# aluo-x/3D_SLN

Measured on AMD Instinct MI355X. Metric: scene-graph VAE steps/sec + 256² diff-render fps, 1/2/4/8 MI355X, higher is better.
Workload: dtype f32; 1 GPU; BASELINE configs[1]: batch=64 scene graphs x (32 objects, 64 triples) per GPU, Sg2ScVAE train step at train.py defaults (embedding_dim=64, 5+5 GraphTripleConv, BatchNorm); O=2048, T=4096, hipgraph=True, distinct_batches_cycled=4, eps=N(0,1) drawn on the device inside the step, parallelism=dp1

## Files before the change

### 3d_sln_amd/_lib.py

```python
from __future__ import annotations

import ctypes as C
import os

HERE = os.path.dirname(os.path.abspath(__file__))
LIB_PATH = os.path.join(HERE, "libsln_hip.so")

SLN_E = {-1: "SLN_E_BADARG", -2: "SLN_E_UNSUPPORTED", -3: "SLN_E_STATE", -4: "SLN_E_NOGPU", -5: "SLN_E_NOMEM", -6: "SLN_E_CAPTURE"}

c_f32p = C.c_void_p
c_i64p = C.c_void_p


class SlnError(RuntimeError):
    pass


class SlnVaeConfig(C.Structure):
    _fields_ = [(n, C.c_int) for n in (
        "embedding_dim", "gconv_num_layers", "recurrent", "batch_norm", "decoder_cat", "use_ae",
        "box_dim", "n_angle", "num_objs", "num_preds", "num_attrs", "no_attr")]


class SlnVaeUnit(C.Structure):
# ... 49 lines not shown
    _fields_ = [("P", SlnPlacement)] + \
               [(n, C.c_void_p) for n in ("boxes", "angles", "size_target", "faces_out", "sizes", "size_loss", "grad_faces", "grad_size_loss",
                                          "grad_boxes", "grad_angles", "boxes_pred", "angles_pred", "noise", "noise_step")] + \
               [("noise_stride", C.c_int64)] + [(n, C.c_void_p) for n in ("box_last", "angle_last", "grad_boxes_pred", "grad_angles_pred")] + \
               [("n_angle", C.c_int), ("ld_gb", C.c_int), ("beta", C.c_float), ("pad_", C.c_int)]


class SlnVaeGroupIO(C.Structure):
    _fields_ = [("rows_total", C.c_int), ("row0_host", C.POINTER(C.c_int))] + \
               [(n, C.c_void_p) for n in ("z", "boxes_pred", "angles_pred", "d_boxes_pred", "d_angles_pred", "dz", "sgd_step")]


class SlnDbgBn(C.Structure):
    _fields_ = [(n, C.c_void_p) for n in ("sums", "gsums", "gamma", "beta", "rmean", "rvar")] + \
               [("cstride", C.c_int), ("mode", C.c_int), ("n_rows", C.c_float), ("eps", C.c_float)]


class SlnDbgSeg(C.Structure):
    _fields_ = [("x1", C.c_void_p), ("x2", C.c_void_p)] + \
               [(n, C.c_int) for n in ("ld1", "ld2", "c1", "c2", "len", "which", "coef", "pad_")] + [("bn", SlnDbgBn)]


class SlnDbgOperand(C.Structure):
    _fields_ = [("seg", SlnDbgSeg * 3), ("idx_a", C.c_void_p), ("idx_b", C.c_void_p), ("nseg", C.c_int), ("pad_", C.c_int)]


class SlnDbgGemmNT(C.Structure):
    _fields_ = [("A", SlnDbgOperand)] + [(n, C.c_void_p) for n in ("W", "bias", "Y", "addend", "xprev", "osums", "ogsums")] + \
               [("obn", SlnDbgBn)] + \
               [(n, C.c_int) for n in ("M", "N", "K", "ldw", "ldy", "ycol0", "ldadd", "addcol0", "ocstride", "ldx", "xcol0", "epi", "tile",
                                       "pad_")]


class SlnDbgGemmTN(C.Structure):
    _fields_ = [("G", SlnDbgOperand), ("X", SlnDbgOperand), ("dW", C.c_void_p), ("db", C.c_void_p), ("sgd_step", C.c_void_p)] + \
               [(n, C.c_int) for n in ("lddw", "R", "Nout", "Kin", "rows_per_block", "pad_")]


class SlnDbgNTRoute(C.Structure):
    _fields_ = [(n, C.c_int) for n in ("body", "multi", "amode", "threads")]


SIGNATURES = {
    "sln_version": (C.c_int, []),
    "sln_build_arch": (C.c_char_p, []),
    "sln_device_ok": (C.c_int, []),
    "sln_vae_num_units": (C.c_int, [C.POINTER(SlnVaeConfig)]),
    "sln_vae_create": (C.c_int, [C.POINTER(SlnVaeConfig), C.POINTER(C.c_void_p)]),
    "sln_vae_destroy": (None, [C.c_void_p]),
    "sln_vae_workspace_bytes": (C.c_int64, [C.c_void_p, C.c_int, C.c_int]),
    "sln_vae_bind": (C.c_int, [C.c_void_p, C.POINTER(SlnVaeTensors), C.c_void_p, C.c_int64, C.c_int, C.c_int]),
    "sln_vae_set_batch": (C.c_int, [C.c_void_p, C.POINTER(SlnVaeBatch), C.c_void_p]),
    "sln_vae_check_batch": (C.c_int, [C.c_void_p, C.c_void_p]),
    "sln_vae_encoder": (C.c_int, [C.c_void_p, c_f32p, c_f32p, C.c_int, C.c_void_p]),
    "sln_vae_decoder": (C.c_int, [C.c_void_p, c_f32p, c_f32p, c_f32p, C.c_int, C.c_void_p]),
    "sln_vae_forward": (C.c_int, [C.c_void_p, c_f32p, c_f32p, c_f32p, c_f32p, c_f32p, c_f32p, C.c_int, C.c_void_p]),
    "sln_vae_loss": (C.c_int, [C.c_void_p, c_f32p, c_f32p, c_f32p, c_f32p, C.c_float, c_f32p, C.c_int, C.c_void_p]),
    "sln_vae_decoder_backward": (C.c_int, [C.c_void_p, c_f32p, c_f32p, c_f32p, C.c_void_p]),
    "sln_vae_encoder_backward": (C.c_int, [C.c_void_p, c_f32p, c_f32p, C.c_void_p]),
    "sln_vae_backward": (C.c_int, [C.c_void_p, C.c_void_p]),
    "sln_vae_params_changed": (C.c_int, [C.c_void_p]),
    "sln_vae_zero_grad": (C.c_int, [C.c_void_p, C.c_void_p]),
    "sln_vae_adam_step": (C.c_int, [C.c_void_p, C.c_float, C.c_void_p]),
    "sln_vae_adam_reset": (C.c_int, [C.c_void_p, C.c_int64, C.c_void_p]),
    "sln_vae_adam_get_step": (C.c_int, [C.c_void_p, C.POINTER(C.c_int64), C.c_void_p]),
    "sln_vae_set_grad_guard": (C.c_int, [C.c_void_p, c_f32p]),
    "sln_vae_seed": (C.c_int, [C.c_void_p, C.c_uint64, C.c_uint64, C.c_void_p]),
    "sln_vae_last_eps": (C.c_int, [C.c_void_p, c_f32p, C.c_void_p]),
    "sln_vae_randn": (C.c_int, [C.c_void_p, c_f32p, C.c_int64, C.c_void_p]),
    "sln_layout_heatmap": (C.c_int, [c_f32p, C.c_int64, C.c_int, C.c_int, C.c_int, C.c_int, c_f32p, C.c_void_p]),
    "sln_vae_set_training": (C.c_int, [C.c_void_p, C.c_int]),
    "sln_vae_train_step": (C.c_int, [C.c_void_p, c_f32p, C.c_float, C.c_float, c_f32p, C.c_int, C.c_int, C.c_void_p]),
    "sln_vae_group_create": (C.c_int, [C.POINTER(C.c_void_p), C.c_int, C.POINTER(SlnVaeGroupIO), C.POINTER(C.c_void_p)]),
    "sln_vae_group_decoder": (C.c_int, [C.c_void_p, C.c_void_p]),
    "sln_vae_group_decoder_backward": (C.c_int, [C.c_void_p, C.c_void_p]),
    "sln_vae_group_launches": (C.c_int, [C.c_void_p, C.POINTER(C.c_int), C.POINTER(C.c_int), C.POINTER(C.c_int)]),
    "sln_vae_group_transposes": (C.c_int64, [C.c_void_p]),
    "sln_vae_group_fused_params": (C.c_int, [C.c_void_p, C.POINTER(C.c_void_p), C.POINTER(C.c_int64), C.c_int]),
    "sln_vae_group_destroy": (None, [C.c_void_p]),
    "sln_debug_side_stream": (C.c_int, [C.c_void_p, C.POINTER(C.c_int), C.POINTER(C.c_int)]),
    "sln_side_stream_prepare": (C.c_int, [C.c_void_p]),
    "sln_side_stream_forget": (C.c_int, [C.c_void_p]),
    "sln_prof_enable": (C.c_int, [C.c_int]),
    "sln_set_deterministic": (C.c_int, [C.c_int]),
    "sln_get_deterministic": (C.c_int, []),
    "sln_debug_tn_plan": (C.c_int, [C.c_void_p, C.c_void_p, C.c_void_p, C.c_int, C.c_void_p, C.c_void_p, C.c_int]),
    "sln_prof_read": (C.c_int, [C.c_void_p, C.c_void_p, C.c_void_p, C.c_int]),
    "sln_vae_tap": (C.c_int64, [C.c_void_p, C.c_int, C.c_int, c_f32p, C.c_void_p]),
    "sln_gconv_workspace_bytes": (C.c_int64, [C.c_int, C.c_int, C.c_int, C.c_int, C.c_int, C.c_int]),
    "sln_gconv_forward": (C.c_int, [C.c_int, C.c_int, C.c_int, C.c_int, C.c_int, C.c_int, C.POINTER(SlnVaeUnit), c_f32p, c_f32p,
                                    C.c_void_p, C.c_int, C.c_int, C.c_int, C.c_void_p, C.c_int64, c_f32p, c_f32p, C.c_void_p]),
    "sln_gconv_net_create": (C.c_int, [C.c_int, C.c_int, C.c_int, C.c_int, C.c_int, C.c_int, C.POINTER(C.c_void_p)]),
    "sln_gconv_net_set_edges": (C.c_int, [C.c_void_p, C.c_void_p, C.c_int, C.c_int, C.c_void_p]),
    "sln_gconv_net_forward": (C.c_int, [C.c_void_p, c_f32p, c_f32p, c_f32p, c_f32p, C.c_int, C.c_void_p]),
    "sln_gconv_net_backward": (C.c_int, [C.c_void_p, c_f32p, c_f32p, c_f32p, c_f32p, C.c_void_p]),
    "sln_linear_forward": (C.c_int, [c_f32p, C.c_int, C.c_int, c_f32p, c_f32p, c_f32p, C.c_int, C.c_void_p,
                                     C.c_int, C.c_void_p]),
    "sln_linear_wgrad": (C.c_int, [c_f32p, c_f32p, C.c_int, C.c_int, C.c_int, c_f32p, c_f32p, C.c_void_p]),
    "sln_debug_gemm_nt": (C.c_int, [C.POINTER(SlnDbgGemmNT), C.c_int, C.POINTER(C.c_int), C.c_void_p]),
    "sln_debug_gemm_tn": (C.c_int, [C.POINTER(SlnDbgGemmTN), C.c_int, C.c_int, C.c_void_p]),
    "sln_debug_gemm_nt_route": (C.c_int, [C.POINTER(SlnDbgGemmNT), C.POINTER(SlnDbgNTRoute)]),
    "sln_debug_gemm_sizes": (C.c_int, [C.POINTER(C.c_int), C.c_int]),
    "sln_project_faces": (C.c_int, [c_f32p, C.c_void_p, c_f32p, c_f32p, c_f32p, C.c_int, C.c_int, C.c_int, C.c_float, C.c_float, c_f32p, C.c_void_p]),
    "sln_project_faces_backward": (C.c_int, [c_f32p, C.c_void_p, c_f32p, c_f32p, c_f32p, C.c_int, C.c_int, C.c_int, C.c_float, C.c_float, c_f32p,
                                             c_f32p, C.c_void_p]),
    "sln_raster_workspace_bytes": (C.c_int64, [C.c_int, C.c_int]),
# ... 143 lines not shown
```

### 3d_sln_amd/csrc/vae_engine.hip

```cpp
#include <cstddef>
#include <new>
#include <type_traits>
#include <utility>
#include <vector>
#include <cstring>
#include <cstdlib>

#include "../../include/sln_hip.h"
#include "sln_gemm.h"
#include "vae_kernels.h"
#include "vae_multi.h"
#include "sln_prof.h"

namespace {

enum { SK_DEC_ASSEMBLE = 0, SK_EMBED_GATHER, SK_NT, SK_SCATTER_FWD, SK_TN, SK_TN_FLUSH, SK_MASK_GSTATS, SK_ADD2, SK_EMBED_BWD,
       SK_SCATTER_BWD, SK_GATHER_BWD, SK_DEC_ASSEMBLE_BWD, SK_COPY2D };
struct RecStep {
  int kind = -1, epi = 0, idx64 = 0;
  GemmNTArgs nt; GemmTNArgs tn;
  MScatterFwd sf; MScatterBwd sb; MGatherBwd gb; MMaskGstats mg; MDecAssemble da; DecAssembleBwd dab; MEmbedGather eg; MEmbedBwd eb; MAdd2 a2;
};
struct Recorder { std::vector<RecStep> steps; };

// ... 32 lines not shown
struct Bump {
  char* base; size_t off = 0; bool dry;
  explicit Bump(void* b) : base(static_cast<char*>(b)), dry(b == nullptr) {}
  template <typename T> T* take(size_t n) {
    off = (off + 255) & ~size_t(255);
    T* p = dry ? nullptr : reinterpret_cast<T*>(base + off);
    off += n * sizeof(T);
    return p;
  }
};

}

struct SlnVae {
  SlnVaeConfig cfg;
  int E, H, L, nmod, n_obj_e, n_attr_e, n_box_e, n_angle_e, Dec, Ddc;
  std::vector<Unit> units;
  SlnVaeTensors t;
  bool bound = false;
  int maxO = 0, maxT = 0, O = 0, T = 0;
  SlnVaeBatch batch;
  bool batch_set = false;

  std::vector<Layer> layers;
  std::vector<BnInst> bns;
  int bn_head[6] = {-1, -1, -1, -1, -1, -1};
  int n_bn_enc = 0;

  GraphCsr g;
  int* attrs32 = nullptr; int* err_flag = nullptr;
  double* stats_base = nullptr; size_t stats_doubles = 0, enc_stats_doubles = 0;
  double* gstats_base = nullptr;
  char* zero_begin = nullptr; size_t zero_bytes = 0; bool bulk_zeroed = false;
  bool step_training = true;
  int64_t* st_objs = nullptr; int64_t* st_angles = nullptr; int64_t* st_attrs = nullptr; float* st_boxes = nullptr;
  BnTableEntry* bn_table_dev = nullptr;
  TransposeEntry* tr_table_dev = nullptr; int n_tr = 0, tr_max_tiles = 0;
  AdamScalars* scalars = nullptr; double* loss_acc = nullptr; float* losses = nullptr;
  float *X0e = nullptr, *P0e = nullptr, *X0d = nullptr, *P0d = nullptr;
  float *hbA1 = nullptr, *hbA2 = nullptr, *haA1 = nullptr, *haA2 = nullptr;
  float *mu = nullptr, *logvar = nullptr, *z = nullptr, *eps_buf = nullptr;
  float *bnA1 = nullptr, *anA1 = nullptr, *boxes_pred = nullptr, *logits = nullptr, *angles_pred = nullptr;
  float *dbp = nullptr, *dlogits = nullptr, *g_bn = nullptr, *g_an = nullptr, *d_bx = nullptr, *d_ax = nullptr;
  float *dM = nullptr, *dG[2] = {nullptr, nullptr};
  float *dX0 = nullptr, *dz = nullptr, *dmu = nullptr, *dlv = nullptr;
  float *g_h2 = nullptr, *g_h1 = nullptr, *d_xb = nullptr, *d_xa = nullptr, *tmp_d = nullptr;
  float *g_h2b = nullptr, *g_h1b = nullptr, *tmp_db = nullptr;
  int dbp_ld = 8;

  bool enc_training = false, dec_training = false, have_enc = false, have_dec = false, have_loss_grads = false;
  const float* z_src = nullptr;
  bool z_from_latent = false;
  bool wt_fresh = false;
  float host_kl = 0.f, host_lr = 0.f; int64_t host_step = 0; bool host_scalars_valid = false;
  float* grad_guard = nullptr;
  bool draw_eps = false;
  unsigned long long host_seed[2] = {0, 0};

  struct TnGroup {
    GemmTNArgs probs[SLN_TN_MULTI_MAX]; TnMultiMeta meta; int n = 0, blocks = 0; bool x2 = false, xg = false; double flops = 0.0;
    bool dirty = true; GemmTNArgs* dev_probs = nullptr; TnMultiMeta* dev_meta = nullptr;
  };
  int tn_slots = 32;
  std::vector<GemmTNArgs> tn_kind_scratch;
  bool capturing = false, tn_upload_pending = false;
  int det_seen = 0;
  bool tn_per_layer = false;
  int tn_slot_next[3] = {0, 0, 0};
  std::vector<GemmTNArgs> deferred;
  TnGroup* tn_groups_store = nullptr;
  TnGroup& tn_group(int set, int slot, int k) { return tn_groups_store[((size_t)set * tn_slots + slot) * 2 + k]; }
  int upload_group(TnGroup& g) {
    hipError_t e = hipMemcpy(g.dev_probs, g.probs, sizeof(GemmTNArgs) * (size_t)g.n, hipMemcpyHostToDevice);
    if (e == hipSuccess) e = hipMemcpy(g.dev_meta, &g.meta, sizeof(TnMultiMeta), hipMemcpyHostToDevice);
    g.dirty = e != hipSuccess;
    return (int)e;
  }
  bool bn_table_live = false;
  struct TnStage { char* host = nullptr; hipEvent_t done = nullptr; };
  enum { TN_STAGE_SLOTS = 16 };
  TnStage tn_stage[TN_STAGE_SLOTS];
  int tn_stage_next = 0;
  int stage_upload(void* dev0, const void* src0, size_t n0, void* dev1, const void* src1, size_t n1, hipStream_t st) {
    hipStreamCaptureStatus cs = hipStreamCaptureStatusNone;
    if (hipStreamIsCapturing(st, &cs) != hipSuccess || cs != hipStreamCaptureStatusNone) return SLN_E_CAPTURE;
    const size_t cap0 = sizeof(GemmTNArgs) * (size_t)SLN_TN_MULTI_MAX, cap = cap0 + sizeof(TnMultiMeta);
    if (n0 > cap0 || n1 > cap - cap0) return SLN_E_BADARG;
    TnStage& sl = tn_stage[tn_stage_next];
    tn_stage_next = (tn_stage_next + 1) % TN_STAGE_SLOTS;
    hipError_t e = hipSuccess;
    if (!sl.host) {
      void* hp = nullptr;
      if (hipHostMalloc(&hp, cap, hipHostMallocDefault) != hipSuccess) return SLN_E_NOMEM;
      sl.host = static_cast<char*>(hp);
      if (hipEventCreateWithFlags(&sl.done, hipEventDisableTiming) != hipSuccess) { (void)hipHostFree(hp); sl.host = nullptr; return SLN_E_NOMEM; }
    } else {
      e = hipEventSynchronize(sl.done);
    }
    if (e == hipSuccess && n0) { std::memcpy(sl.host, src0, n0); e = hipMemcpyAsync(dev0, sl.host, n0, hipMemcpyHostToDevice, st); }
    if (e == hipSuccess && n1) { std::memcpy(sl.host + cap0, src1, n1); e = hipMemcpyAsync(dev1, sl.host + cap0, n1, hipMemcpyHostToDevice, st); }
    if (e == hipSuccess) e = hipEventRecord(sl.done, st);
    return (int)e;
  }
  int upload_group_async(TnGroup& g, hipStream_t st) {
    const int r = stage_upload(g.dev_probs, g.probs, sizeof(GemmTNArgs) * (size_t)g.n, g.dev_meta, &g.meta,
                               offsetof(TnMultiMeta, item) + sizeof(TnMultiItem) * (size_t)g.meta.nblocks, st);
// ... 834 lines not shown
  }
  h->n_tr = (int)tr.size(); h->tr_max_tiles = maxt;
  HIP_RET(hipMemcpy(h->tr_table_dev, tr.data(), sizeof(TransposeEntry) * tr.size(), hipMemcpyHostToDevice));
  AdamScalars sc; std::memset(&sc, 0, sizeof(sc));
  sc.step = 0; sc.lr = 1e-4f; sc.beta1 = 0.9f; sc.beta2 = 0.999f; sc.eps = 1e-8f; sc.kl_weight = 0.1f; sc.bc1 = 1.f; sc.bc2 = 1.f;
  sc.rng_seed = h->host_seed[0]; sc.rng_offset = h->host_seed[1];
  HIP_RET(hipMemcpy(h->scalars, &sc, sizeof(sc), hipMemcpyHostToDevice));
  RET_IF(sln_gemm_init());
  h->host_scalars_valid = false;
  h->bound = true; h->batch_set = false; h->wt_fresh = false; h->have_enc = h->have_dec = false; h->bn_table_live = false;
  h->drop_graphs();
  return 0;
}

static int upload_bn_table(SlnVae* h) {
  std::vector<BnTableEntry> tab(h->bns.size());
  for (size_t i = 0; i < h->bns.size(); ++i) {
    BnInst& b = h->bns[i];
    const Unit& u = h->units[b.unit];
    BnTableEntry e; std::memset(&e, 0, sizeof(e));
    e.sums = b.sums; e.gsums = b.gsums; e.cstride = b.C; e.C = b.C; e.rows = b.rows_code;
    e.rmean = u.p.bn_running_mean; e.rvar = u.p.bn_running_var; e.nbt = u.p.bn_num_batches_tracked;
    e.dgamma = u.p.d_bn_weight; e.dbeta = u.p.d_bn_bias;
    tab[i] = e;
  }
  if (!tab.empty()) HIP_RET(hipMemcpy(h->bn_table_dev, tab.data(), sizeof(BnTableEntry) * tab.size(), hipMemcpyHostToDevice));
  return 0;
}

int sln_vae_set_batch(SlnVae* h, const SlnVaeBatch* b, void* stream) {
  if (!h || !b || !h->bound) return SLN_E_BADARG;
  if (b->O <= 0 || b->T < 0 || b->O > h->maxO || b->T > h->maxT) return SLN_E_BADARG;
  if (!b->objs || !b->boxes || !b->angles || !b->attributes || (b->T > 0 && !b->triples)) return SLN_E_BADARG;
  hipStream_t st = (hipStream_t)stream;
  const bool shape_changed = (b->O != h->O) || (b->T != h->T) || !h->batch_set;
  h->batch = *b; h->O = b->O; h->T = b->T;
  h->g.T = b->T; h->g.O = b->O;
  if (shape_changed) {
    for (auto& ly : h->layers)
      for (int k = 0; k < 4; ++k)
        if (ly.bn[k] >= 0) h->bns[ly.bn[k]].rows = k < 2 ? b->T : b->O;
    for (int s = 0; s < 6; ++s)
      if (h->bn_head[s] >= 0) h->bns[h->bn_head[s]].rows = b->O;
    if (!h->bn_table_live) {
      HIP_RET(hipStreamSynchronize(st));
      RET_IF(upload_bn_table(h));
      h->bn_table_live = true;
    }
    bool has_graph = false;
    for (int i = 0; i < 4; ++i) has_graph |= h->graph_exec[i] != nullptr;
    if (has_graph) HIP_RET(hipStreamSynchronize(st));
    h->drop_graphs();
  }
  RET_IF(sln_zero_async(h->err_flag, sizeof(int), st));
  StageBatch sb; std::memset(&sb, 0, sizeof(sb));
  sb.objs = b->objs; sb.attrs = b->attributes; sb.angles = b->angles; sb.boxes = b->boxes;
  sb.st_objs = h->st_objs; sb.st_attrs = h->st_attrs; sb.st_angles = h->st_angles; sb.st_boxes = h->st_boxes;
  sb.attrs32 = h->attrs32; sb.deg = h->g.deg; sb.err = h->err_flag;
  sb.O = b->O; sb.box_dim = h->cfg.box_dim; sb.n_objs = h->cfg.num_objs; sb.n_attrs = h->cfg.num_attrs; sb.n_angle = h->cfg.n_angle;
  RET_IF(sln_launch_stage_batch(sb, st));
  h->batch.objs = h->st_objs; h->batch.angles = h->st_angles; h->batch.attributes = h->st_attrs; h->batch.boxes = h->st_boxes;
  RET_IF(sln_launch_graph_prep(b->triples, b->T, b->O, h->cfg.num_preds, h->g, h->err_flag, st, 0, 1));
  h->batch_set = true; h->have_enc = h->have_dec = false;
  return 0;
}

int sln_vae_check_batch(SlnVae* h, void* stream) {
  if (!h || !h->batch_set) return SLN_E_STATE;
  int flag = 0;
  HIP_RET(hipMemcpyAsync(&flag, h->err_flag, sizeof(int), hipMemcpyDeviceToHost, (hipStream_t)stream));
  HIP_RET(hipStreamSynchronize((hipStream_t)stream));
  return flag ? SLN_E_BADARG : 0;
}

static int copy_out(float* dst, const float* src, size_t n, hipStream_t st) {
  if (!dst || dst == src) return 0;
  return (int)hipMemcpyAsync(dst, src, n * sizeof(float), hipMemcpyDeviceToDevice, st);
}

int sln_vae_encoder(SlnVae* h, float* mu, float* logvar, int training, void* stream) {
  if (!h || !h->batch_set) return SLN_E_STATE;
  hipStream_t st = (hipStream_t)stream;
  RET_IF(h->encoder_forward(training != 0, st));
  RET_IF(copy_out(mu, h->mu, (size_t)h->O * h->E, st));
  RET_IF(copy_out(logvar, h->logvar, (size_t)h->O * h->E, st));
  return 0;
}

int sln_vae_decoder(SlnVae* h, const float* z, float* boxes_pred, float* angles_pred, int training, void* stream) {
  if (!h || !h->batch_set) return SLN_E_STATE;
  if (!z) return SLN_E_BADARG;
  hipStream_t st = (hipStream_t)stream;
  RET_IF(h->decoder_forward(z, nullptr, training != 0, st));
  RET_IF(copy_out(boxes_pred, h->boxes_pred, (size_t)h->O * h->cfg.box_dim, st));
  RET_IF(copy_out(angles_pred, h->angles_pred, (size_t)h->O * h->cfg.n_angle, st));
  return 0;
}

int sln_vae_forward(SlnVae* h, const float* eps, float* mu, float* logvar, float* z_out, float* boxes_pred,
                    float* angles_pred, int training, void* stream) {
  if (!h || !h->batch_set) return SLN_E_STATE;
  hipStream_t st = (hipStream_t)stream;
  if (eps) RET_IF(copy_out(h->eps_buf, eps, (size_t)h->O * h->E, st));
  else if (!h->cfg.use_ae) RET_IF(sln_launch_randn(h->eps_buf, (long)h->O * h->E, h->scalars, st));
  RET_IF(h->encoder_forward(training != 0, st));
  RET_IF(h->decoder_forward(nullptr, h->eps_buf, training != 0, st));
  RET_IF(copy_out(mu, h->mu, (size_t)h->O * h->E, st));
  RET_IF(copy_out(logvar, h->logvar, (size_t)h->O * h->E, st));
  RET_IF(copy_out(z_out, h->z, (size_t)h->O * h->E, st));
  RET_IF(copy_out(boxes_pred, h->boxes_pred, (size_t)h->O * h->cfg.box_dim, st));
  RET_IF(copy_out(angles_pred, h->angles_pred, (size_t)h->O * h->cfg.n_angle, st));
  return 0;
}

static int set_kl(SlnVae* h, float kl_weight, float lr, hipStream_t st) {
  if (kl_weight != h->host_kl || !h->host_scalars_valid) {
    h->host_kl = kl_weight;
// ... 798 lines not shown
```

### 3d_sln_amd/csrc/vae_kernels.h

```cpp
#pragma once
#include "sln_common.h"

struct GraphCsr {
  int* s;
  int* p;
  int* o;
  int* deg;
  float* invdeg;
  int* rowptr;
  int* cursor;
  int* ent;
  int T, O;
};
int sln_launch_graph_prep(const int64_t* triples, int T, int O, int num_preds, GraphCsr g, int* err_flag, hipStream_t st,
                          int edges_only = 0, int deg_is_zero = 0);
int sln_launch_bn_relu_apply(const float* x, int ld, int col0, int cols, int rows, BnView bn, float* out, int ldo, hipStream_t st);
struct StageBatch {
  const int64_t* objs; const int64_t* attrs; const int64_t* angles; const float* boxes;
  int64_t* st_objs; int64_t* st_attrs; int64_t* st_angles; float* st_boxes;
  int* attrs32; int* deg; int* err;
  int O, box_dim, n_objs, n_attrs, n_angle;
};
int sln_launch_stage_batch(const StageBatch& a, hipStream_t st);
int sln_launch_validate_ids(const int64_t* objs, const int64_t* attrs, const int64_t* angles, int O, int n_objs, int n_attrs,
                            int n_angle, int* err_flag, hipStream_t st);

int sln_launch_scatter_avg_fwd(const float* A2, int ld, int H, int D, BnView bn2, GraphCsr g, int O,
                               float* pooled, hipStream_t st);

int sln_launch_scatter_avg_bwd(const float* dM, const float* dP, int lddp, int dpcol0, const float* A2, int ld,
                               int H, int D, BnView bn2, GraphCsr g, int T, float* g2, double* gsums,
                               int cstride, hipStream_t st);

int sln_launch_gather_bwd(const float* dG, int ldg, int D, GraphCsr g, int O, const float* add1, int ldadd1,
                          const float* xprev, int ldx, BnView bn, int masked, float* out, int ldo,
                          double* gsums, int cstride, hipStream_t st);

int sln_launch_add2(const float* a, int lda, const float* b, int ldb, int rows, int cols, float* out, int ldo, hipStream_t st);
int sln_launch_mask_gstats(const float* d1, int ld1, const float* d2, int ld2, const float* xprev, int ldx,
                           BnView bn, int rows, int cols, float* out, int ldo, double* gsums, int cstride,
                           hipStream_t st);

struct EncAssemble {
  const int64_t* objs; const int64_t* attrs; const int64_t* angles; const float* boxes;
  const float* obj_emb; const float* attr_emb; const float* angle_emb; const float* wb; const float* bb;
  int O, n_obj, n_attr, n_box, n_angle, box_dim;
  float* x0;
};
int sln_launch_enc_assemble(EncAssemble a, hipStream_t st);
struct EncAssembleBwd {
  const int64_t* objs; const int64_t* attrs; const int64_t* angles; const float* boxes;
  const float* dx0; int O, n_obj, n_attr, n_box, n_angle, box_dim;
  float* d_obj_emb; float* d_attr_emb; float* d_angle_emb; float* d_wb; float* d_bb;
  int rows_obj, rows_attr, rows_angle;
};
int sln_launch_enc_assemble_bwd(EncAssembleBwd a, hipStream_t st);

struct DecAssemble {
  const int64_t* objs; const int64_t* attrs;
  const float* obj_emb; const float* attr_emb; const float* mu; const float* logvar; const float* eps;
  const float* z_in;
  int O, n_obj, n_attr, n_z, use_ae;
  float* z; float* x0;
  int z_in_x0;
};
int sln_launch_dec_assemble(DecAssemble a, hipStream_t st);
struct DecAssembleBwd {
  const int64_t* objs; const int64_t* attrs; const float* dx0; int O, n_obj, n_attr, n_z;
  float* d_obj_emb; float* d_attr_emb; float* dz;
  int z_in_x0;
  int rows_obj, rows_attr;
};
int sln_launch_dec_assemble_bwd(DecAssembleBwd a, hipStream_t st);

int sln_launch_embed_gather_i32(const int* idx, const float* emb, int rows, int n, float* out, hipStream_t st);
int sln_launch_embed_bwd_i32(const int* idx, const float* d, int ld, int col0, int rows, int n, int table_rows,
// ... 56 lines not shown
```

### 3d_sln_amd/csrc/vae_kernels.hip

```cpp
#include <cstring>
#include "vae_kernels.h"
#include "sln_prof.h"

namespace {

constexpr int CB = 64;
constexpr int RL = 4;
constexpr int BOX_ROWS = 64;
constexpr int RB = 32;

__device__ __forceinline__ void commit_col_stats(float s1, float s2, bool valid, double* out, int cstride, int col) {
  __shared__ float red[2][RL][CB];
  red[0][threadIdx.y][threadIdx.x] = s1;
  red[1][threadIdx.y][threadIdx.x] = s2;
  __syncthreads();
  if (threadIdx.y == 0 && valid && out != nullptr) {
    float a = 0.f, b = 0.f;
#pragma unroll
    for (int i = 0; i < RL; ++i) { a += red[0][i][threadIdx.x]; b += red[1][i][threadIdx.x]; }
    atomicAdd(out + col, sln_qd((double)a, SLN_Q_BWD));
    atomicAdd(out + cstride + col, sln_qd((double)b, SLN_Q_BWD));
  }
}

// ... 820 lines not shown
                                     float* __restrict__ out, int ldo) {
  const long i = (long)blockIdx.x * blockDim.x + threadIdx.x;
  if (i >= n) return;
  const long r = i / cols; const int c = (int)(i % cols);
  float sc, sh;
  bn_fwd_coef(bn, c, sc, sh);
  out[r * ldo + c] = fmaxf(fmaf(sc, x[r * ld + col0 + c], sh), 0.f);
}

__device__ __forceinline__ void add2_body(const float* __restrict__ a, int lda, const float* __restrict__ b, int ldb, int rows, int cols,
                            float* __restrict__ out, int ldo) {
  const long i = (long)blockIdx.x * blockDim.x + threadIdx.x;
  if (i >= (long)rows * cols) return;
  const int r = (int)(i / cols), c = (int)(i % cols);
  out[(size_t)r * ldo + c] = a[(size_t)r * lda + c] + b[(size_t)r * ldb + c];
}
__global__ void add2_kernel(const float* __restrict__ a, int lda, const float* __restrict__ b, int ldb, int rows, int cols, float* __restrict__ out, int ldo) {
  add2_body(a, lda, b, ldb, rows, cols, out, ldo);
}

inline dim3 colgrid(int cols, int rows) { return dim3(sln_cdiv(cols, CB), sln_cdiv(rows, RB)); }

}

__global__ void validate_ids_kernel(const int64_t* __restrict__ objs, const int64_t* __restrict__ attrs,
                                    const int64_t* __restrict__ angles, int O, int n_objs, int n_attrs, int n_angle, int* err) {
  const int i = blockIdx.x * blockDim.x + threadIdx.x;
  if (i >= O) return;
  if (objs[i] < 0 || objs[i] >= n_objs) atomicOr(err, 2);
  if (attrs[i] < 0 || attrs[i] >= n_attrs) atomicOr(err, 4);
  if (angles && (angles[i] < 0 || angles[i] >= n_angle)) atomicOr(err, 8);
}

__global__ void stage_batch_kernel(StageBatch a) {
  const int i = blockIdx.x * blockDim.x + threadIdx.x;
  if (i >= a.O) return;
  const int64_t ob = a.objs[i], at = a.attrs[i], an = a.angles[i];
  a.st_objs[i] = ob; a.st_attrs[i] = at; a.st_angles[i] = an;
  a.attrs32[i] = (int)at;
  a.deg[i] = 0;
  for (int k = 0; k < a.box_dim; ++k) a.st_boxes[(size_t)i * a.box_dim + k] = a.boxes[(size_t)i * a.box_dim + k];
  if (ob < 0 || ob >= a.n_objs) atomicOr(a.err, 2);
  if (a.n_attrs > 0 && (at < 0 || at >= a.n_attrs)) atomicOr(a.err, 4);
  if (an < 0 || an >= a.n_angle) atomicOr(a.err, 8);
}

int sln_launch_stage_batch(const StageBatch& a, hipStream_t st) {
  if (a.O <= 0) return 0;
  hipLaunchKernelGGL(stage_batch_kernel, dim3(sln_cdiv(a.O, 256)), dim3(256), 0, st, a);
  SLN_CHECK_LAUNCH();
  return 0;
}

int sln_launch_validate_ids(const int64_t* objs, const int64_t* attrs, const int64_t* angles, int O, int n_objs, int n_attrs,
                            int n_angle, int* err_flag, hipStream_t st) {
  if (O <= 0) return 0;
  hipLaunchKernelGGL(validate_ids_kernel, dim3(sln_cdiv(O, 256)), dim3(256), 0, st, objs, attrs, angles, O, n_objs, n_attrs, n_angle,
                     err_flag);
  SLN_CHECK_LAUNCH();
  return 0;
}

int sln_launch_graph_prep(const int64_t* triples, int T, int O, int num_preds, GraphCsr g, int* err_flag, hipStream_t st,
                          int edges_only, int deg_is_zero) {
  if (!deg_is_zero) {
    const int e = sln_zero_async(g.deg, sizeof(int) * (size_t)O, st);
    if (e != 0) return e;
  }
  if (T > 0) hipLaunchKernelGGL(prep_split_kernel, dim3(sln_cdiv(T, 256)), dim3(256), 0, st, triples, T, O, num_preds, g, err_flag,
                              edges_only ? 2 : 3, edges_only ? -1 : 1, edges_only ? 1 : 2);
  hipLaunchKernelGGL(csr_scan_kernel, dim3(1), dim3(1024), 0, st, g, O);
  if (T > 0) hipLaunchKernelGGL(csr_fill_kernel, dim3(sln_cdiv(2 * T, 256)), dim3(256), 0, st, g, T);
  hipLaunchKernelGGL(csr_sort_kernel, dim3(O), dim3(64), 0, st, g, O);
  SLN_CHECK_LAUNCH();
  return 0;
}

int sln_launch_bn_relu_apply(const float* x, int ld, int col0, int cols, int rows, BnView bn, float* out, int ldo, hipStream_t st) {
  const long n = (long)rows * cols;
  if (n <= 0) return 0;
  hipLaunchKernelGGL(bn_relu_apply_kernel, dim3((unsigned)((n + 255) / 256)), dim3(256), 0, st, x, ld, col0, cols, n, bn, out, ldo);
  SLN_CHECK_LAUNCH();
  return 0;
}

int sln_launch_scatter_avg_fwd(const float* A2, int ld, int H, int D, BnView bn2, GraphCsr g, int O, float* pooled,
                               hipStream_t st) {
  if (O <= 0) return 0;
  { static const int a = std::getenv("SLN_EDGE_ABL") ? std::atoi(std::getenv("SLN_EDGE_ABL")) : 0; if (a & 1) return 0; }
  SlnProfScope prof(SLN_FAM_EDGE, 4.0 * g.T * 2 * H + 4.0 * O * H + 16.0 * g.T, st);
  if (H % 4 == 0 && D % 4 == 0 && ld % 4 == 0 && al16(A2) && al16(pooled)) {
    if (H > 128) hipLaunchKernelGGL((scatter_avg_fwd_v4_kernel<64, 4>), dim3(sln_cdiv(H, 256), sln_cdiv(O, 4)), dim3(64, 4), 0, st, A2, ld, H, D, bn2, g, O, g.T, pooled);
    else hipLaunchKernelGGL((scatter_avg_fwd_v4_kernel<32, 8>), dim3(sln_cdiv(H, 128), sln_cdiv(O, 8)), dim3(32, 8), 0, st, A2, ld, H, D, bn2, g, O, g.T, pooled);
    SLN_CHECK_LAUNCH();
    return 0;
  }
  return -2;
}

int sln_launch_scatter_avg_bwd(const float* dM, const float* dP, int lddp, int dpcol0, const float* A2, int ld, int H,
                               int D, BnView bn2, GraphCsr g, int T, float* g2, double* gsums, int cstride,
                               hipStream_t st) {
  if (T <= 0) return 0;
  { static const int a = std::getenv("SLN_EDGE_ABL") ? std::atoi(std::getenv("SLN_EDGE_ABL")) : 0; if (a & 2) return 0; }
  SlnProfScope prof(SLN_FAM_EDGE, 4.0 * T * (2 * H) + (dP ? 4.0 * T * D : 0.0) + 2.0 * 4.0 * T * (2 * H + D) + 8.0 * T, st);
  if (H % 4 == 0 && D % 4 == 0 && ld % 4 == 0 && (!dP || (lddp % 4 == 0 && dpcol0 % 4 == 0 && al16(dP))) && al16(dM) && al16(A2) && al16(g2)) {
// ... 614 lines not shown
```

### include/sln_hip.h

```cpp
#ifndef SLN_HIP_H
#define SLN_HIP_H

#include <stdint.h>

#ifdef __cplusplus
extern "C" {
#endif

#define SLN_E_BADARG (-1)
#define SLN_E_UNSUPPORTED (-2)
#define SLN_E_STATE (-3)
#define SLN_E_NOGPU (-4)
#define SLN_E_NOMEM (-5)
#define SLN_E_CAPTURE (-6)

int sln_version(void);
const char* sln_build_arch(void);
int sln_device_ok(void);


typedef struct SlnVaeConfig {
  int embedding_dim;
  int gconv_num_layers;
  int recurrent;
  int batch_norm;
  int decoder_cat;
  int use_ae;
  int box_dim;
  int n_angle;
  int num_objs;
  int num_preds;
  int num_attrs;
  int no_attr;
} SlnVaeConfig;

int sln_vae_num_units(const SlnVaeConfig* cfg);

typedef struct SlnVaeUnit {
  float* weight;  float* bias;
  float* bn_weight; float* bn_bias;
  float* bn_running_mean; float* bn_running_var; int64_t* bn_num_batches_tracked;
  float* d_weight; float* d_bias; float* d_bn_weight; float* d_bn_bias;
} SlnVaeUnit;

typedef struct SlnVaeTensors {
  float* obj_emb_ec;  float* d_obj_emb_ec;
  float* pred_emb_ec; float* d_pred_emb_ec;
  float* obj_emb_dc;  float* d_obj_emb_dc;
  float* pred_emb_dc; float* d_pred_emb_dc;
  float* attr_emb_ec; float* d_attr_emb_ec;
  float* attr_emb_dc; float* d_attr_emb_dc;
  float* box_emb_w;   float* d_box_emb_w;
  float* box_emb_b;   float* d_box_emb_b;
  float* angle_emb;   float* d_angle_emb;
  const SlnVaeUnit* units_host;
  float* flat_params; float* flat_grads; float* adam_m; float* adam_v; int64_t n_flat;
} SlnVaeTensors;

typedef struct SlnVaeBatch {
  const int64_t* objs;
  const int64_t* triples;
  const float*   boxes;
  const int64_t* angles;
  const int64_t* attributes;
  int O, T;
} SlnVaeBatch;

typedef struct SlnVae SlnVae;

int sln_vae_create(const SlnVaeConfig* cfg, SlnVae** out);
void sln_vae_destroy(SlnVae* h);
int64_t sln_vae_workspace_bytes(const SlnVae* h, int max_objs, int max_triples);
int sln_vae_bind(SlnVae* h, const SlnVaeTensors* t, void* workspace, int64_t workspace_bytes,
                 int max_objs, int max_triples);

int sln_vae_set_batch(SlnVae* h, const SlnVaeBatch* b, void* stream);
int sln_vae_check_batch(SlnVae* h, void* stream);

int sln_vae_encoder(SlnVae* h, float* mu, float* logvar, int training, void* stream);
int sln_vae_decoder(SlnVae* h, const float* z, float* boxes_pred, float* angles_pred, int training, void* stream);
int sln_vae_forward(SlnVae* h, const float* eps, float* mu, float* logvar, float* z_out, float* boxes_pred,
                    float* angles_pred, int training, void* stream);

int sln_vae_loss(SlnVae* h, const float* boxes_pred, const float* angles_pred, const float* mu,
                 const float* logvar, float kl_weight, float* losses_out, int with_grads, void* stream);

int sln_vae_decoder_backward(SlnVae* h, const float* d_boxes_pred, const float* d_angles_pred, float* dz, void* stream);
int sln_vae_encoder_backward(SlnVae* h, const float* d_mu, const float* d_logvar, void* stream);
int sln_vae_backward(SlnVae* h, void* stream);

int sln_vae_params_changed(SlnVae* h);
int sln_vae_zero_grad(SlnVae* h, void* stream);
int sln_vae_adam_step(SlnVae* h, float lr, void* stream);
int sln_vae_adam_reset(SlnVae* h, int64_t step, void* stream);
int sln_vae_adam_get_step(SlnVae* h, int64_t* step_out, void* stream);
int sln_vae_set_grad_guard(SlnVae* h, float* slot);
int sln_vae_seed(SlnVae* h, uint64_t seed, uint64_t offset, void* stream);
int sln_vae_last_eps(SlnVae* h, float* eps_out, void* stream);
int sln_vae_randn(SlnVae* h, float* out, int64_t n, void* stream);
int sln_layout_heatmap(const float* boxes_pred, int64_t n_trials, int O, int box_dim, int container_size, int clip_coor, float* counts,
                       void* stream);

enum { SLN_TRAIN_BACKWARD = 0, SLN_TRAIN_FULL = 1, SLN_TRAIN_UPTO_DECODER = 2, SLN_TRAIN_ENCODER_BWD = 3 };
int sln_vae_set_training(SlnVae* h, int training);
int sln_vae_train_step(SlnVae* h, const float* eps, float kl_weight, float lr, float* losses_out, int use_graph,
                       int with_adam, void* stream);

typedef struct SlnVaeGroup SlnVaeGroup;
typedef struct SlnVaeGroupIO {
  int rows_total;
  const int* row0_host;
  const float* z;
  float* boxes_pred;
  float* angles_pred;
  float* d_boxes_pred;
  float* d_angles_pred;
  float* dz;
  const float* sgd_step;
} SlnVaeGroupIO;
int sln_vae_group_create(SlnVae* const* engines, int R, const SlnVaeGroupIO* io, SlnVaeGroup** out);
int sln_vae_group_decoder(SlnVaeGroup* g, void* stream);
int sln_vae_group_decoder_backward(SlnVaeGroup* g, void* stream);
int sln_vae_group_fused_params(const SlnVaeGroup* g, const float** params, int64_t* numel, int max);
int sln_vae_group_launches(const SlnVaeGroup* g, int* fwd, int* bwd, int* single_room_fallbacks);
int64_t sln_vae_group_transposes(const SlnVaeGroup* g);
void sln_vae_group_destroy(SlnVaeGroup* g);

int sln_debug_side_stream(void* stream, int* index, int* overlapped);
int sln_side_stream_prepare(void* stream);
int sln_side_stream_forget(void* stream);
// ... 277 lines not shown
```

Baseline: 34720 graphs/s (scene-graph VAE fwd+loss+bwd+Adam).

## Fuse batch staging and graph CSR prep into one single-block bind kernel

When a batch fits in shared-memory limits (O≤2048, T≤4096), set_batch now launches one kernel that copies and validates the batch, counts degrees, scans them into rowptr, and builds the sorted edge list in shared memory. This replaces the err-flag memset, the stage kernel and the multi-kernel graph prep. The aim is to cut launch count and global-memory round trips per step. In exchange, the CSR build is serialised onto one 1024-thread block, with a quadratic per-node rank sort that could be slow for high-degree nodes. Debug hooks to force or inspect the path are added.

```diff
diff --git a/3d_sln_amd/_lib.py b/3d_sln_amd/_lib.py
--- a/3d_sln_amd/_lib.py
+++ b/3d_sln_amd/_lib.py
@@ -125,6 +125,8 @@
     "sln_vae_bind": (C.c_int, [C.c_void_p, C.POINTER(SlnVaeTensors), C.c_void_p, C.c_int64, C.c_int, C.c_int]),
     "sln_vae_set_batch": (C.c_int, [C.c_void_p, C.POINTER(SlnVaeBatch), C.c_void_p]),
     "sln_vae_check_batch": (C.c_int, [C.c_void_p, C.c_void_p]),
+    "sln_debug_vae_bind_path": (C.c_int, [C.c_void_p, C.c_int]),
+    "sln_debug_vae_bind_read": (C.c_int64, [C.c_void_p, C.c_int, C.c_void_p, C.c_int64, C.c_void_p]),
     "sln_vae_encoder": (C.c_int, [C.c_void_p, c_f32p, c_f32p, C.c_int, C.c_void_p]),
     "sln_vae_decoder": (C.c_int, [C.c_void_p, c_f32p, c_f32p, c_f32p, C.c_int, C.c_void_p]),
     "sln_vae_forward": (C.c_int, [C.c_void_p, c_f32p, c_f32p, c_f32p, c_f32p, c_f32p, c_f32p, C.c_int, C.c_void_p]),
diff --git a/3d_sln_amd/csrc/vae_engine.hip b/3d_sln_amd/csrc/vae_engine.hip
--- a/3d_sln_amd/csrc/vae_engine.hip
+++ b/3d_sln_amd/csrc/vae_engine.hip
@@ -108,6 +108,7 @@
   const float* z_src = nullptr;
   bool z_from_latent = false;
   bool wt_fresh = false;
+  int bind_force = -1, bind_path = -1;
   float host_kl = 0.f, host_lr = 0.f; int64_t host_step = 0; bool host_scalars_valid = false;
   float* grad_guard = nullptr;
   bool draw_eps = false;
@@ -1048,17 +1049,45 @@
     if (has_graph) HIP_RET(hipStreamSynchronize(st));
     h->drop_graphs();
   }
-  RET_IF(sln_zero_async(h->err_flag, sizeof(int), st));
   StageBatch sb; std::memset(&sb, 0, sizeof(sb));
   sb.objs = b->objs; sb.attrs = b->attributes; sb.angles = b->angles; sb.boxes = b->boxes;
   sb.st_objs = h->st_objs; sb.st_attrs = h->st_attrs; sb.st_angles = h->st_angles; sb.st_boxes = h->st_boxes;
   sb.attrs32 = h->attrs32; sb.deg = h->g.deg; sb.err = h->err_flag;
   sb.O = b->O; sb.box_dim = h->cfg.box_dim; sb.n_objs = h->cfg.num_objs; sb.n_attrs = h->cfg.num_attrs; sb.n_angle = h->cfg.n_angle;
-  RET_IF(sln_launch_stage_batch(sb, st));
+  const bool fits = sln_bind_batch_fits(b->O, b->T) != 0;
+  if (h->bind_force == 1 && !fits) return SLN_E_BADARG;
+  h->bind_path = h->bind_force >= 0 ? h->bind_force : (fits ? 1 : 0);
+  if (h->bind_path == 1) {
+    BindBatch bb; std::memset(&bb, 0, sizeof(bb));
+    bb.s = sb; bb.triples = b->triples; bb.g = h->g; bb.T = b->T; bb.num_preds = h->cfg.num_preds;
+    RET_IF(sln_launch_bind_batch(bb, st));
+  } else {
+    RET_IF(sln_zero_async(h->err_flag, sizeof(int), st));
+    RET_IF(sln_launch_stage_batch(sb, st));
+    RET_IF(sln_launch_graph_prep(b->triples, b->T, b->O, h->cfg.num_preds, h->g, h->err_flag, st, 0, 1));
+  }
   h->batch.objs = h->st_objs; h->batch.angles = h->st_angles; h->batch.attributes = h->st_attrs; h->batch.boxes = h->st_boxes;
-  RET_IF(sln_launch_graph_prep(b->triples, b->T, b->O, h->cfg.num_preds, h->g, h->err_flag, st, 0, 1));
   h->batch_set = true; h->have_enc = h->have_dec = false;
   return 0;
+}
+
+int sln_debug_vae_bind_path(SlnVae* h, int force) {
+  if (!h || force < -1 || force > 1) return SLN_E_BADARG;
+  h->bind_force = force;
+  return h->bind_path;
+}
+
+int64_t sln_debug_vae_bind_read(SlnVae* h, int which, void* dst, int64_t bytes, void* stream) {
+  if (!h || !h->batch_set) return SLN_E_STATE;
+  const size_t O = (size_t)h->O, T = (size_t)h->T;
+  const void* src[14] = {h->g.s, h->g.p, h->g.o, h->g.deg, h->g.invdeg, h->g.rowptr, h->g.cursor, h->g.ent, h->attrs32, h->err_flag,
+                         h->st_objs, h->st_attrs, h->st_angles, h->st_boxes};
+  const size_t n[14] = {4 * T, 4 * T, 4 * T, 4 * O, 4 * O, 4 * (O + 1), 4 * O, 8 * T, 4 * O, 4, 8 * O, 8 * O, 8 * O, 4 * O * (size_t)h->cfg.box_dim};
+  if (which < 0 || which >= 14) return SLN_E_BADARG;
+  if (!dst) return (int64_t)n[which];
+  if (bytes != (int64_t)n[which]) return SLN_E_BADARG;
+  if (n[which]) HIP_RET(hipMemcpyAsync(dst, src[which], n[which], hipMemcpyDeviceToDevice, (hipStream_t)stream));
+  return (int64_t)n[which];
 }
 
 int sln_vae_check_batch(SlnVae* h, void* stream) {
diff --git a/3d_sln_amd/csrc/vae_kernels.h b/3d_sln_amd/csrc/vae_kernels.h
--- a/3d_sln_amd/csrc/vae_kernels.h
+++ b/3d_sln_amd/csrc/vae_kernels.h
@@ -22,6 +22,10 @@
   int O, box_dim, n_objs, n_attrs, n_angle;
 };
 int sln_launch_stage_batch(const StageBatch& a, hipStream_t st);
+constexpr int SLN_BIND_MAX_O = 2048, SLN_BIND_MAX_T = 4096, SLN_BIND_THREADS = 1024;
+struct BindBatch { StageBatch s; const int64_t* triples; GraphCsr g; int T, num_preds; };
+int sln_bind_batch_fits(int O, int T);
+int sln_launch_bind_batch(const BindBatch& a, hipStream_t st);
 int sln_launch_validate_ids(const int64_t* objs, const int64_t* attrs, const int64_t* angles, int O, int n_objs, int n_attrs,
                             int n_angle, int* err_flag, hipStream_t st);
 
diff --git a/3d_sln_amd/csrc/vae_kernels.hip b/3d_sln_amd/csrc/vae_kernels.hip
--- a/3d_sln_amd/csrc/vae_kernels.hip
+++ b/3d_sln_amd/csrc/vae_kernels.hip
@@ -896,6 +896,91 @@
   return 0;
 }
 
+__device__ __forceinline__ bool bind_triple(const int64_t* __restrict__ tri, int t, int O, int num_preds, int& s, int& p, int& o) {
+  const int64_t s64 = tri[3 * (size_t)t], p64 = tri[3 * (size_t)t + 1], o64 = tri[3 * (size_t)t + 2];
+  if (s64 < 0 || s64 >= O || o64 < 0 || o64 >= O || p64 < 0 || p64 >= num_preds) { s = p = o = 0; return false; }
+  s = (int)s64; p = (int)p64; o = (int)o64;
+  return true;
+}
+static_assert(SLN_BIND_MAX_O <= 2 * SLN_BIND_THREADS, "the scan gives a thread two rows");
+__global__ __launch_bounds__(SLN_BIND_THREADS) void bind_batch_kernel(BindBatch a) {
+  const int tid = threadIdx.x, O = a.s.O, T = a.T;
+  if (blockIdx.x > 0) {
+    const int i = (int)(blockIdx.x - 1) * SLN_BIND_THREADS + tid;
+    if (i >= O) return;
+    const int64_t at = a.s.attrs[i];
+    a.s.st_objs[i] = a.s.objs[i]; a.s.st_attrs[i] = at; a.s.st_angles[i] = a.s.angles[i];
+    a.s.attrs32[i] = (int)at;
+    for (int k = 0; k < a.s.box_dim; ++k) a.s.st_boxes[(size_t)i * a.s.box_dim + k] = a.s.boxes[(size_t)i * a.s.box_dim + k];
+    return;
+  }
+  __shared__ int cur[SLN_BIND_MAX_O + 1], rowp[SLN_BIND_MAX_O + 1], ent[2 * SLN_BIND_MAX_T], part[SLN_BIND_THREADS];
+  __shared__ int flag;
+  for (int i = tid; i <= O; i += SLN_BIND_THREADS) cur[i] = 0;
+  if (tid == 0) flag = 0;
+  __syncthreads();
+  int bad = 0;
+  for (int t = tid; t < T; t += SLN_BIND_THREADS) {
+    int s, p, o;
+    if (!bind_triple(a.triples, t, O, a.num_preds, s, p, o)) bad |= 1;
+    a.g.s[t] = s; a.g.p[t] = p; a.g.o[t] = o;
+    atomicAdd(&cur[s], 1); atomicAdd(&cur[o], 1);
+  }
+  for (int i = tid; i < O; i += SLN_BIND_THREADS) {
+    const int64_t ob = a.s.objs[i], at = a.s.attrs[i], an = a.s.angles[i];
+    if (ob < 0 || ob >= a.s.n_objs) bad |= 2;
+    if (a.s.n_attrs > 0 && (at < 0 || at >= a.s.n_attrs)) bad |= 4;
+    if (an < 0 || an >= a.s.n_angle) bad |= 8;
+  }
+  if (bad) atomicOr(&flag, bad);
+  __syncthreads();
+  const int i0 = 2 * tid, d0 = i0 < O ? cur[i0] : 0, d1 = i0 + 1 < O ? cur[i0 + 1] : 0;
+  part[tid] = d0 + d1;
+  __syncthreads();
+  for (int off = 1; off < SLN_BIND_THREADS; off <<= 1) {
+    const int v = tid >= off ? part[tid - off] : 0;
+    __syncthreads();
+    part[tid] += v;
+    __syncthreads();
+  }
+  const int ex0 = part[tid] - d0 - d1, ex1 = ex0 + d0;
+  if (i0 < O) {
+    cur[i0] = rowp[i0] = ex0;
+    a.g.rowptr[i0] = ex0; a.g.cursor[i0] = ex0 + d0; a.g.deg[i0] = d0; a.g.invdeg[i0] = 1.0f / (float)(d0 > 1 ? d0 : 1);
+  }
+  if (i0 + 1 < O) {
+    cur[i0 + 1] = rowp[i0 + 1] = ex1;
+    a.g.rowptr[i0 + 1] = ex1; a.g.cursor[i0 + 1] = ex1 + d1; a.g.deg[i0 + 1] = d1; a.g.invdeg[i0 + 1] = 1.0f / (float)(d1 > 1 ? d1 : 1);
+  }
+  if (tid == SLN_BIND_THREADS - 1) { rowp[O] = part[tid]; a.g.rowptr[O] = part[tid]; }
+  __syncthreads();
+  for (int e = tid; e < 2 * T; e += SLN_BIND_THREADS) {
+    int s, p, o;
+    bind_triple(a.triples, e < T ? e : e - T, O, a.num_preds, s, p, o);
+    ent[atomicAdd(&cur[e < T ? s : o], 1)] = e;
+  }
+  __syncthreads();
+  for (int k = tid; k < 2 * T; k += SLN_BIND_THREADS) {
+    const int e = ent[k];
+    int s, p, o;
+    bind_triple(a.triples, e < T ? e : e - T, O, a.num_preds, s, p, o);
+    const int node = e < T ? s : o, b = rowp[node], en = rowp[node + 1];
+    int rank = 0;
+    for (int j = b; j < en; ++j) rank += ent[j] < e ? 1 : 0;
+    a.g.ent[b + rank] = e;
+  }
+  if (tid == 0) a.s.err[0] = flag;
+}
+
+int sln_bind_batch_fits(int O, int T) { return O >= 1 && O <= SLN_BIND_MAX_O && T >= 0 && T <= SLN_BIND_MAX_T; }
+
+int sln_launch_bind_batch(const BindBatch& a, hipStream_t st) {
+  if (!sln_bind_batch_fits(a.s.O, a.T) || a.g.O != a.s.O || a.g.T != a.T) return -1;
+  hipLaunchKernelGGL(bind_batch_kernel, dim3(1 + sln_cdiv(a.s.O, SLN_BIND_THREADS)), dim3(SLN_BIND_THREADS), 0, st, a);
+  SLN_CHECK_LAUNCH();
+  return 0;
+}
+
 int sln_launch_validate_ids(const int64_t* objs, const int64_t* attrs, const int64_t* angles, int O, int n_objs, int n_attrs,
                             int n_angle, int* err_flag, hipStream_t st) {
   if (O <= 0) return 0;
diff --git a/include/sln_hip.h b/include/sln_hip.h
--- a/include/sln_hip.h
+++ b/include/sln_hip.h
@@ -76,6 +76,8 @@
 
 int sln_vae_set_batch(SlnVae* h, const SlnVaeBatch* b, void* stream);
 int sln_vae_check_batch(SlnVae* h, void* stream);
+int sln_debug_vae_bind_path(SlnVae* h, int force);
+int64_t sln_debug_vae_bind_read(SlnVae* h, int which, void* dst, int64_t bytes, void* stream);
 
 int sln_vae_encoder(SlnVae* h, float* mu, float* logvar, int training, void* stream);
 int sln_vae_decoder(SlnVae* h, const float* z, float* boxes_pred, float* angles_pred, int training, void* stream);
```

Measured after the change: 34830 graphs/s (scene-graph VAE fwd+loss+bwd+Adam) (median of 6 runs). No clear change (+0.3%).
